# 10XGenomics/supernova

Hardware: AMD Instinct MI355X
Metric: Gk-mers/s through count+graph at k=48, 1.2B×150bp; bit-exact counts (higher is better)
Workload: dtype u64

## Files before the change

supernova_amd/csrc/snk_ctx.h:

```cpp
#pragma once
#include <hip/hip_runtime.h>
#include <stdarg.h>
#include <stdio.h>
#include <string.h>

#include <initializer_list>
#include <string>
#include <vector>

#include "../../include/snk.h"
#include "snk_launch.h"
#include "snk_opts.h"
#include "snk_plan.h"

struct snk_ctx {
    int device = 0;
    hipStream_t stream = nullptr;
    hipStream_t cur_stream = nullptr;
    int n_cu = 256;
    size_t lds_per_block = 65536;
    uint64_t device_mem_total = 0;
    double pass_sigma = 0.0;
    uint64_t plan_mapped = 0;
    uint64_t plan_mem = 0;
// ... 23 lines not shown
    uint32_t last_ovf = 0, last_ovf_nb = 0;
    uint64_t last_ovf_reads = 0;
    uint64_t last_dense = 0;
    uint32_t count_screen = 0;
    uint32_t count_tight = 0;
    snk_sizing_history sizing;
    uint32_t mlen = 16;
    uint32_t last_extra = 0;
    uint64_t last_input_fp = 0;
    bool have_input_fp = false;
    uint32_t last_count_limit = 0;
    uint32_t last_partition_passes = 1;
    uint32_t last_hbv_flood = 0;
    uint64_t last_hbv_dev_components = 0, last_hbv_host_components = 0;
    uint32_t last_bl_attempts = 0, last_bl_big_chunks = 0;
    uint64_t last_bl_circles = 0;
    std::vector<unsigned long long> h_region_off;
    snk_opts opts;
    void* shard = nullptr;
    void* host_io = nullptr;
    void (*host_io_free)(void*) = nullptr;
    void* df_io = nullptr;
    void (*df_io_free)(void*) = nullptr;
    void* stream_job = nullptr;
    void (*stream_job_free)(void*) = nullptr;
    void (*stream_job_invalidate)(void*) = nullptr;
    void* shard_host = nullptr;
    void (*shard_host_free)(void*) = nullptr;
};

// ... 54 lines not shown
```

supernova_amd/csrc/snk_dist.hip:

```cpp
#include <string.h>

#include <vector>

#include "snk_ctx.h"
#include "snk_common.h"
#include "snk_graph.h"
#include "snk_kernels.h"
#include "snk_stages.h"
#include "snk_shard.h"

static snk_shard_state* state_of(snk_ctx* ctx) { return snk_shard_state_of(ctx); }
void snk_shard_state_free(void* p) { delete static_cast<snk_shard_state*>(p); }
void snk_shard_state_invalidate_job(void* p) { if (p) static_cast<snk_shard_state*>(p)->job_open = false; }

int snk_shard_begin(snk_ctx* ctx, const snk_dev_reads* in, const snk_params* p, uint32_t rank, uint32_t world, uint32_t NB_total,
                    uint64_t* n_instances, hipStream_t st, char* err, size_t errcap) {
    if (!ctx || !in || !p) return snk_fail(SNK_E_ARG, err, errcap, "snk_shard_hist: NULL argument");
    if (p->K != 48 && p->K != 60) return snk_fail(SNK_E_UNSUPPORTED, err, errcap, "K=%u is not supported (48 or 60)", p->K);
    if (p->min_bc > 8) return snk_fail(SNK_E_UNSUPPORTED, err, errcap, "min_bc=%u: the device barcode rule tells up to eight distinct barcodes apart (min_bc <= 8)", p->min_bc);
    if (world == 0 || rank >= world || NB_total == 0 || NB_total % world) return snk_fail(SNK_E_ARG, err, errcap, "snk_shard_hist: NB_total must be a positive multiple of world");
    if (world > 0x7FFF) return snk_fail(SNK_E_UNSUPPORTED, err, errcap, "world > 32767");
    if (in->n_reads && (!in->rows || in->row_words * 16 < in->read_len || in->read_len > 256 || (!in->quals && !in->good_len)))
        return snk_fail(SNK_E_ARG, err, errcap, "snk_shard_hist: bad reads");
    SNK_HIP_TRY(snk_enter(ctx));
    snk_ctx_release_scratch(ctx);
    snk_shard_state* S = state_of(ctx);
    S->reads = *in;
    S->params = *p;
    S->rank = rank; S->world = world; S->NB_total = NB_total; S->NBl = NB_total / world;
    S->circ_all = nullptr; S->join_circles = 0;
    ctx->last_bl_attempts = ctx->last_bl_big_chunks = 0; ctx->last_bl_circles = 0;
    const uint16_t* good_len = (const uint16_t*)in->good_len;
    int rc;
    const bool fused = in->n_reads && snk_fused_trim_ok(ctx, in);
    snk_fused_trim ft;
    if (!good_len) {
        void* gl;
        if ((rc = snk_ctx_alloc(ctx, in->n_reads * 2 + 2, &gl, err, errcap))) return rc;
        if (fused) { ft.quals = in->quals; ft.qstride = in->qstride; ft.lens = in->lens; ft.min_qual = p->min_qual; ft.good_out = (uint16_t*)gl; }
        else if (in->n_reads) {
            rc = snk_dev_trim(ctx, in->quals, in->qstride, in->lens, in->read_len, in->n_reads, p->K, p->min_qual, gl, st);
            if (rc) return snk_fail(rc, err, errcap, "%s", snk_last_error());
        }
        good_len = (const uint16_t*)gl;
    }
    S->good_len = good_len;
// ... 13 lines not shown
int snk_shard_job_open(snk_ctx* ctx, const snk_params* p, uint32_t rank, uint32_t world, uint32_t NB_total, uint32_t read_len, uint64_t reads_ub,
                       uint64_t total_reads, int has_bc, hipStream_t st, char* err, size_t errcap) {
    if (!ctx || !p) return snk_fail(SNK_E_ARG, err, errcap, "snk_shard_stream_begin: NULL argument");
    if (p->K != 48 && p->K != 60) return snk_fail(SNK_E_UNSUPPORTED, err, errcap, "K=%u is not supported (48 or 60)", p->K);
    if (p->min_bc > 8) return snk_fail(SNK_E_UNSUPPORTED, err, errcap, "min_bc=%u: the device barcode rule tells up to eight distinct barcodes apart (min_bc <= 8)", p->min_bc);
    if (world == 0 || rank >= world || NB_total == 0 || NB_total % world) return snk_fail(SNK_E_ARG, err, errcap, "snk_shard_stream_begin: NB_total must be a positive multiple of world");
    if (read_len == 0 || read_len > 256 || reads_ub == 0) return snk_fail(SNK_E_ARG, err, errcap, "snk_shard_stream_begin: read_len 1..256 and an upper bound of this rank's reads are needed");
    SNK_HIP_TRY(snk_enter(ctx));
    snk_ctx_release_scratch(ctx);
    snk_shard_state* S = state_of(ctx);
    memset(&S->reads, 0, sizeof S->reads);
    S->params = *p;
    S->rank = rank; S->world = world; S->NB_total = NB_total; S->NBl = NB_total / world;
    S->circ_all = nullptr; S->join_circles = 0;
    ctx->last_bl_attempts = ctx->last_bl_big_chunks = 0; ctx->last_bl_circles = 0;
    S->job_open = false; S->job_read_len = read_len; S->job_has_bc = has_bc; S->job_reads_ub = reads_ub; S->job_total_reads = total_reads;
    void* q;
    int rc;
    if ((rc = snk_ctx_alloc(ctx, 64, &q, err, errcap))) return rc; S->status = (uint32_t*)q;
    SNK_HIP_TRY(hipMemsetAsync(S->status, 0, 64, st));
    if ((rc = snk_ctx_alloc(ctx, reads_ub * 2 + 64, &q, err, errcap))) return rc; S->job_good_len = (uint16_t*)q;
    const unsigned long long kpr = read_len >= p->K ? read_len - p->K + 1 : 0;
    if ((rc = snk_partition_open(ctx, st, p->K, NB_total, reads_ub * kpr, reads_ub, false, S->status, &S->job, err, errcap))) return rc;
    S->job_open = true;
    return SNK_OK;
}
int snk_shard_job_add(snk_ctx* ctx, const snk_dev_reads* slab, hipStream_t st, char* err, size_t errcap) {
    if (!ctx || !ctx->shard || !slab) return snk_fail(SNK_E_ARG, err, errcap, "snk_shard_stream_append: NULL argument / no open step");
    snk_shard_state* S = state_of(ctx);
    if (!S->job_open) return snk_fail(SNK_E_ARG, err, errcap, "snk_shard_stream_append: no open step (snk_shard_stream_begin)");
// ... 569 lines not shown
```

supernova_amd/csrc/snk_local.hip:

```cpp
#include <string.h>
#include <cstring>
#include <rocprim/rocprim.hpp>

#include <type_traits>

#include "snk_ctx.h"
#include "snk_common.h"
#include "snk_kernels.h"
#include "snk_graph.h"
#include "snk_stages.h"

namespace {

constexpr uint32_t NONE = 0xFFFFFFFFu;
constexpr unsigned long long NONE64 = ~0ull;
constexpr uint16_t NONE16 = 0xFFFFu;
constexpr int TB = 256;

struct chunk_src {
    const uint32_t* chunk_n;
    const uint32_t* chunk_base;
    const uint4* extra;
    const unsigned long long* region_off;
    uint32_t NB, n_extra, n_regions;
// ... 46 lines not shown
        const uint4 e = cs.extra[c - cs.NB];
        bucket = e.x; off = e.y; n = e.z & 0xFFFu; region = e.z >> 12; meta = e.w;
    }
    const uint64_t base = cs.region_off[region] + off;
    desc[c] = make_uint4((uint32_t)base, n, bucket, meta);
    if (desc_src) desc_src[c] = (uint64_t)region * region_cap + off;
}
__device__ __forceinline__ chunk_t chunk_get(const uint4* __restrict__ desc, uint32_t c) {
    const uint4 d = desc[c];
    chunk_t k;
    k.base = d.x; k.n = d.y; k.bucket = d.z; k.lg = d.w >> 24; k.id = d.w & 0xFFFFFFu; k.span = 1;
    if (d.w >> 31) { k.lg = 0; k.id = 0; k.span = d.w & 0xFFFFu; }
    return k;
}

__device__ __forceinline__ snk_kmer load_key(const snk_u128* keys, uint64_t i) {
    const uint64_t* p = reinterpret_cast<const uint64_t*>(keys + i);
    snk_kmer k;
    k.lo = p[0];
    k.hi = p[1];
    return k;
}
__device__ __forceinline__ uint32_t lhash(uint64_t hi, uint64_t lo) {
    uint32_t x = (uint32_t)(hi >> 32) * 0x9E3779B1u ^ (uint32_t)hi * 0x85EBCA77u ^ (uint32_t)(lo >> 32) * 0xC2B2AE3Du ^
                 (uint32_t)lo * 0x27D4EB2Fu;
    return snk_mix32(x);
}
template <int K>
__device__ __forceinline__ uint32_t oriented_base(snk_kmer k, bool rc, int idx) {
    return rc ? (snk_kmer_base<K>(k, K - 1 - idx) ^ 3u) : snk_kmer_base<K>(k, idx);
}

template <int K, int CAP, int T, bool BIG, bool GR, int MM>
__device__ __forceinline__ void bl_prune_chunk(const uint32_t c, const uint4* __restrict__ desc, uint32_t NB, bl_shard sh, const bl_regions& rg,
                                                     const snk_u128* __restrict__ keys, const uint64_t* __restrict__ vals,
                                                     uint32_t do_prune, uint8_t* __restrict__ ctx_out,
                                                     uint32_t* __restrict__ count_out, uint8_t* __restrict__ pend_out,
                                                     uint32_t* __restrict__ nbr_out, uint32_t* __restrict__ nbnd,
                                                     uint32_t* __restrict__ biglist, uint32_t* __restrict__ nbig,
                                                     unsigned long long* __restrict__ gindex, uint64_t gmask) {
    constexpr int HT = CAP <= 256 ? 512 : 4096;
    typedef typename std::conditional<(K <= 48 && !GR), uint32_t, uint64_t>::type klo_w;
    constexpr int KLS = (K <= 48 && !GR) ? 32 : 0;
    __shared__ uint64_t khi[CAP];
    __shared__ klo_w klo[CAP];
    __shared__ uint32_t ht[HT];
    __shared__ uint32_t bcnt;
    const int tid = threadIdx.x;
    const chunk_t ch = chunk_get(desc, c);
    if (ch.n == 0) return;
    if (!BIG && ch.n > (uint32_t)CAP) {
        if (tid == 0) biglist[atomicAdd(nbig, 1u)] = c;
        return;
    }
    const uint32_t n = ch.n;
// ... 23 lines not shown
            if (rg.keys_r) { uint64_t* d = reinterpret_cast<uint64_t*>(rg.keys_dense + ch.base + i); d[0] = kq[q].lo; d[1] = kq[q].hi; }
        }
    }
    __syncthreads();
    for (uint32_t i = tid; i < n; i += T) {
        uint32_t slot = lhash(khi[i], (uint64_t)klo[i] << KLS) & (HT - 1);
        for (;;) {
            const uint32_t old = atomicCAS(&ht[slot], 0u, i + 1u);
            if (old == 0u) break;
            slot = (slot + 1) & (HT - 1);
        }
    }
    __syncthreads();
    const uint32_t split_mask = (1u << ch.lg) - 1u;
    uint32_t mybnd = 0;
    __shared__ uint16_t mlist[8 * T];
    __shared__ uint32_t resL[T];
    __shared__ uint32_t mcnt;
#pragma unroll
    for (int q = 0; q < NPT; ++q) {
        const uint32_t i0 = q * T;
        if (i0 >= n) break;
        const uint32_t i = i0 + tid;
        const bool act = i < n;
        snk_kmer k;
        k.hi = act ? khi[i] : 0ull;
        k.lo = act ? ((uint64_t)klo[i] << KLS) : 0ull;
        uint64_t tag = 0;
        if (GR) { tag = k.lo & 0xFFFFFFFFull; k.lo &= ~0xFFFFFFFFull; }
        const uint64_t v = myv[q];
// ... 78 lines not shown
                    snk_kmer cn = snk_kmer_lt(r, y) ? r : y;
                    if (GR) cn.lo |= ktag;
                    uint32_t h1, h2;
                    snk_kmer_hash_count<(K > 48) || GR>(cn, &h1, &h2);
                    here = (h2 & split_mask) == ch.id;
                }
                if (here && !(do_prune & 2u)) { if (!(do_prune & 1u)) atomicOr(&resL[th], 1u << bit); }
                else atomicOr(&resL[th], (1u << bit) | (0x100u << bit) | (remote ? (0x10000u << bit) : 0u));
            }
        }
        __syncthreads();
        const uint32_t res = resL[tid];
        keep |= res & 0xFFu;
        const uint32_t pm = (res >> 8) & 0xFFu;
        __syncthreads();
        if (!act) continue;
        const uint64_t gi = ch.base + i;
        ctx_out[gi] = (uint8_t)keep;
        pend_out[gi] = (uint8_t)pm;
        if (sh.premote) sh.premote[gi] = (uint8_t)(res >> 16);
        count_out[gi] = (uint32_t)(v >> 8);
        nbr_out[gi] = (nb0 == NONE ? 0x0FFFu : nb0) | (snk_kmer_eq(k, kr) ? 0x8000u : 0u) | ((nb1 == NONE ? 0x0FFFu : nb1) << 16);
        if (pm) {
            ++mybnd;
            if (gindex) {
                snk_kmer kk;
                kk.hi = khi[i];
                kk.lo = (uint64_t)klo[i] << KLS;
                uint32_t h1, h2;
                snk_kmer_hash2(kk, &h1, &h2);
                uint64_t slot = (((uint64_t)h1 << 32) | h2) & gmask;
                const unsigned long long ent = ((unsigned long long)h1 << 32) | (unsigned long long)(gi + 1);
                if (gindex[gmask + 1] == 0ull) {
                    bool placed = false;
                    for (uint32_t tries = 0; tries < 64; ++tries) {
                        const unsigned long long old = atomicCAS(&gindex[slot], 0ull, ent);
                        if (old == 0ull) { placed = true; break; }
                        slot = (slot + 1) & gmask;
                    }
                    if (!placed) gindex[gmask + 1] = 1ull;
                }
            }
        }
    }
    snk_wave_add(&bcnt, mybnd);
    __syncthreads();
    if (tid == 0) nbnd[c] = bcnt;
}
template <int K, int CAP, int T, bool BIG, bool GR, int MM>
__global__ void __launch_bounds__(T) bl_prune_kernel(const uint4* __restrict__ desc, uint32_t NB, bl_shard sh, bl_regions rg, const uint32_t* __restrict__ biglist_in,
                                                     uint32_t nchunks, uint32_t cpw,
                                                     const snk_u128* __restrict__ keys, const uint64_t* __restrict__ vals,
                                                     uint32_t do_prune, uint8_t* __restrict__ ctx_out,
                                                     uint32_t* __restrict__ count_out, uint8_t* __restrict__ pend_out,
                                                     uint32_t* __restrict__ nbr_out, uint32_t* __restrict__ nbnd,
                                                     uint32_t* __restrict__ biglist, uint32_t* __restrict__ nbig, const uint32_t* __restrict__ n_dev,
                                                     unsigned long long* __restrict__ gindex, uint64_t gmask) {
    if (BIG && n_dev) {
        const uint32_t nb = *n_dev;
        for (uint32_t w = blockIdx.x; w < nb; w += gridDim.x)
            bl_prune_chunk<K, CAP, T, BIG, GR, MM>(biglist_in[w], desc, NB, sh, rg, keys, vals, do_prune, ctx_out, count_out, pend_out, nbr_out, nbnd, biglist, nbig, gindex, gmask);
        return;
    }
    for (uint32_t r = 0; r < cpw; ++r) {
        const uint32_t w = blockIdx.x * cpw + r;
        if (w >= nchunks) return;
        bl_prune_chunk<K, CAP, T, BIG, GR, MM>(BIG ? biglist_in[w] : w, desc, NB, sh, rg, keys, vals, do_prune, ctx_out, count_out, pend_out, nbr_out,
                                       nbnd, biglist, nbig, gindex, gmask);
    }
}

__global__ void __launch_bounds__(TB) bl_index_build_kernel(const snk_u128* __restrict__ keys, const uint8_t* __restrict__ pend,
                                                            uint64_t n, unsigned long long* __restrict__ tab, uint64_t mask) {
    const uint64_t i = (uint64_t)blockIdx.x * TB + threadIdx.x;
    if (i >= n || !pend[i]) return;
    const snk_kmer k = load_key(keys, i);
    uint32_t h1, h2;
    snk_kmer_hash2(k, &h1, &h2);
    uint64_t slot = (((uint64_t)h1 << 32) | h2) & mask;
    const unsigned long long ent = ((unsigned long long)h1 << 32) | (unsigned long long)(i + 1);
    for (;;) {
        const unsigned long long old = atomicCAS(&tab[slot], 0ull, ent);
        if (old == 0ull) break;
        slot = (slot + 1) & mask;
    }
}
template <int K, bool GR>
__global__ void __launch_bounds__(TB) bl_resolve_kernel(const snk_u128* __restrict__ keys, const uint8_t* __restrict__ pend,
                                                        uint64_t n, const unsigned long long* __restrict__ tab, uint64_t mask,
                                                        uint32_t do_prune, uint8_t* __restrict__ ctx, uint32_t* __restrict__ rq,
                                                        const uint8_t* __restrict__ premote) {
    constexpr int SPAN = 8 * TB;
    __shared__ uint16_t list[SPAN];
    __shared__ uint32_t cnt;
    const uint64_t base = (uint64_t)blockIdx.x * SPAN;
    if (threadIdx.x == 0) cnt = 0;
    __syncthreads();
    {
        const uint64_t i8 = base + 8ull * threadIdx.x;
        unsigned long long w = 0;
        if (i8 + 8 <= n) w = *reinterpret_cast<const unsigned long long*>(pend + i8);
        else for (uint64_t q = i8; q < n; ++q) w |= (unsigned long long)pend[q] << (8 * (q - i8));
        if (w) {
            uint32_t m = 0;
            for (int q = 0; q < 8; ++q) if ((w >> (8 * q)) & 0xFFull) ++m;
            uint32_t pos = atomicAdd(&cnt, m);
            for (int q = 0; q < 8; ++q) if ((w >> (8 * q)) & 0xFFull) list[pos++] = (uint16_t)(8 * threadIdx.x + q);
        }
    }
    __syncthreads();
    const uint32_t m = cnt;
    for (uint32_t it = threadIdx.x; it < m; it += TB) {
        const uint64_t i = base + list[it];
        const uint32_t pm = pend[i] & (premote ? ~(uint32_t)premote[i] : 0xFFu);
        snk_kmer k = load_key(keys, i);
        uint64_t tag = 0;
        if (GR) { tag = k.lo & 0xFFFFFFFFull; k.lo &= ~0xFFFFFFFFull; }
        uint32_t c = ctx[i];
        const snk_kmer kr = snk_kmer_rc<K>(k);
        for (uint32_t rem = pm; rem; rem &= rem - 1) {
            const uint32_t bit = __ffs(rem) - 1;
            const snk_kmer y = bit < 4 ? snk_kmer_succ<K>(k, bit) : snk_kmer_pred<K>(k, bit - 4);
            const snk_kmer r = bit < 4 ? snk_kmer_pred<K>(kr, 3u - bit) : snk_kmer_succ<K>(kr, 7u - bit);
            const bool rev = snk_kmer_lt(r, y);
            snk_kmer cy = rev ? r : y;
            if (GR) cy.lo |= tag;
            uint32_t h1, h2;
            snk_kmer_hash2(cy, &h1, &h2);
            uint64_t slot = (((uint64_t)h1 << 32) | h2) & mask;
            int64_t j = -1;
            for (;;) {
                const unsigned long long e = tab[slot];
                if (e == 0ull) break;
                if ((uint32_t)(e >> 32) == h1) {
                    const uint64_t idx = (uint32_t)e - 1u;
                    if (snk_kmer_eq(load_key(keys, idx), cy)) { j = (int64_t)idx; break; }
                }
                slot = (slot + 1) & mask;
            }
            if (j >= 0) rq[2 * i + (bit >> 2)] = ((uint32_t)j << 1) | (rev ? 1u : 0u);
            else if (do_prune) c &= ~(1u << bit);
            else rq[2 * i + (bit >> 2)] = NONE;
        }
        ctx[i] = (uint8_t)c;
    }
}

struct bl_extra_pool {
    unsigned long long* cur;
    uint64_t f0, b0;
    uint64_t fcap, bcap;
};
struct bl_dist_args {
    const uint8_t* premote;
    const uint32_t* rq_idx;
    const uint16_t* rq_meta;
    const unsigned long long* node_off;
    unsigned long long my_node_off;
};
template <int K, int CAP, int T, bool BIG, bool EMIT, bool DIST, bool GR>
// ... 420 lines not shown
    B->premote = nullptr;
    if (B->world > 1 || B->force_dist) {
        G_ALLOC(B->premote, uint8_t, n + 16);
        SNK_HIP_TRY(hipMemsetAsync(B->premote, 0, n + 16, st));
    }
    SNK_HIP_TRY(hipMemsetAsync(nbnd, 0, ((uint64_t)nchunks + 1) * 4, st));
    SNK_HIP_TRY(hipMemsetAsync(ctr, 0, 64, st));
    bl_shard sh;
    sh.bucket_base = B->premote ? B->rank * B->NBl : 0u;
    sh.NBl = B->premote ? B->NBl : 0u;
    sh.me = B->rank;
    sh.G = tab->n_regions ? tab->n_regions : 1u;
    sh.premote = B->premote;
    const uint32_t NBh = B->premote ? B->NB_total : tab->NB;
    const uint32_t cpw = snk_opt_u32(ctx, SNK_OPT_bl_cpw);
    uint64_t tg0 = 0;
    unsigned long long* index0 = nullptr;
    if (snk_opt_u32(ctx, SNK_OPT_bl_index_fused)) {
        const uint64_t guess = (ctx->last_bnd_n == n && ctx->last_bnd) ? ctx->last_bnd + ctx->last_bnd / 8 : n / 5;
        tg0 = 1024;
        while (tg0 < 2 * guess) tg0 <<= 1;
        G_ALLOC(index0, unsigned long long, tg0 + 1);
        SNK_HIP_TRY(hipMemsetAsync(index0, 0, (tg0 + 1) * 8, st));
    }
    bl_regions rg;
    rg.keys_r = tab->keys_r; rg.vals_r = tab->vals_r; rg.desc_src = desc_src;
    rg.keys_dense = const_cast<snk_u128*>(tab->keys);
    const bool long_m = ctx->mlen == (uint32_t)SNK_M_LONG;
    SNK_HIP_TRY(snk_launch(long_m ? bl_prune_kernel<K, SCAP, ST, false, GR, SNK_M_LONG> : bl_prune_kernel<K, SCAP, ST, false, GR, SNK_M_OF(K)>, snk_blocks(nchunks, cpw), ST, 0, st, (const uint4*)B->desc, NBh, sh, rg,
                           (const uint32_t*)nullptr, nchunks, cpw, tab->keys, tab->vals, B->do_prune | (snk_opt_u32(ctx, SNK_OPT_bl_noclassify) ? 2u : 0u), B->ctx, B->counts, B->pend, B->nbr, nbnd,
                           B->biglist, ctr, (const uint32_t*)nullptr, index0, tg0 - 1));
    uint32_t h_nbig = 0;
    SNK_HIP_TRY(hipMemcpyAsync(ctr + 1, ctr, 4, hipMemcpyDeviceToDevice, st));
    SNK_HIP_TRY(snk_launch(long_m ? bl_prune_kernel<K, BCAP, BT, true, GR, SNK_M_LONG> : bl_prune_kernel<K, BCAP, BT, true, GR, SNK_M_OF(K)>, 2048, BT, 0, st, (const uint4*)B->desc, NBh, sh, rg,
                           (const uint32_t*)B->biglist, 0u, 1u, tab->keys, tab->vals, B->do_prune | (snk_opt_u32(ctx, SNK_OPT_bl_noclassify) ? 2u : 0u), B->ctx, B->counts, B->pend, B->nbr,
                           nbnd, B->biglist, ctr + 2, (const uint32_t*)(ctr + 1), index0, tg0 - 1));
    if (tab->keys_r) {
        snk_ctx_release_block(ctx, tab->keys_r);
        snk_ctx_release_block(ctx, tab->vals_r);
    }
    unsigned long long* d_sum;
    G_ALLOC(d_sum, unsigned long long, 2);
    {
        size_t tb = 0;
        auto in = rocprim::make_transform_iterator(nbnd, [] __device__(uint32_t v) { return (unsigned long long)v; });
        SNK_HIP_TRY(rocprim::reduce((void*)nullptr, tb, in, d_sum, 0ull, (size_t)nchunks, rocprim::plus<unsigned long long>(), st));
        void* tmp;
        int rc = snk_ctx_alloc(ctx, tb, &tmp, err, errcap);
        if (rc) return rc;
        SNK_HIP_TRY(rocprim::reduce(tmp, tb, in, d_sum, 0ull, (size_t)nchunks, rocprim::plus<unsigned long long>(), st));
    }
    unsigned long long h_bnd = 0, h_gaveup = 0;
    if (index0) SNK_HIP_TRY(hipMemcpyAsync(&h_gaveup, index0 + tg0, 8, hipMemcpyDeviceToHost, st));
    SNK_HIP_TRY(hipMemcpyAsync(&h_bnd, d_sum, 8, hipMemcpyDeviceToHost, st));
    SNK_HIP_TRY(hipMemcpyAsync(&h_nbig, ctr + 1, 4, hipMemcpyDeviceToHost, st));
    SNK_HIP_TRY(snk_sync(st));
    B->nbig = h_nbig;
    B->n_boundary = h_bnd;
    ctx->last_bnd = h_bnd; ctx->last_bnd_n = n;
    uint64_t tg = 1024;
    while (tg < 2 * h_bnd) tg <<= 1;
    const bool fused_ok = index0 && !h_gaveup && h_bnd * 4 <= tg0 * 3;
    if (fused_ok) { B->index = index0; tg = tg0; }
    else {
        if (index0) snk_ctx_release_block(ctx, index0);
        G_ALLOC(B->index, unsigned long long, tg);
        SNK_HIP_TRY(hipMemsetAsync(B->index, 0, tg * 8, st));
    }
    B->index_mask = tg - 1;
    if (h_bnd) {
        if (!fused_ok) SNK_HIP_TRY(snk_launch(bl_index_build_kernel, snk_blocks(n, TB), TB, 0, st, tab->keys, B->pend, n, B->index, tg - 1));
        SNK_HIP_TRY(snk_launch(bl_resolve_kernel<K, GR>, snk_blocks(n, 8 * TB), TB, 0, st, tab->keys, B->pend, n,
                               B->index, tg - 1, B->do_prune, B->ctx, B->rq, (const uint8_t*)B->premote));
    }
    return SNK_OK;
}

template <int K, bool DIST, bool GR>
static int bl_fragments_impl(snk_ctx* ctx, hipStream_t st, snk_bl_state* B, const bl_dist_args& da, snk_frag_out* out, char* err,
                             size_t errcap) {
    const snk_table* tab = B->tab;
    const uint32_t nchunks = B->nchunks, h_nbig = B->nbig;
    uint32_t *nfrag, *foff;
    uint64_t *nbases, *boff;
    G_ALLOC(nfrag, uint32_t, (uint64_t)nchunks + 1);
    G_ALLOC(foff, uint32_t, (uint64_t)nchunks + 1);
    G_ALLOC(nbases, uint64_t, (uint64_t)nchunks + 1);
    G_ALLOC(boff, uint64_t, (uint64_t)nchunks + 1);
    SNK_HIP_TRY(hipMemsetAsync(nfrag, 0, ((uint64_t)nchunks + 1) * 4, st));
// ... 224 lines not shown
```

supernova_amd/csrc/snk_opts.hip:

```cpp
#include <stdio.h>
#include <stdlib.h>
#include <string.h>

#include <string>

#include "snk_opts.h"
#ifndef SNK_OPTS_NO_CTX
#include "snk_ctx.h"
#endif

const snk_opt_def snk_opt_defs[SNK_OPT_COUNT] = {
#define X(name, dflt, range, doc) {#name, dflt, range, doc},
    SNK_OPTIONS(X)
#undef X
};

int snk_opt_index(const char* name) {
    if (!name) return -1;
    for (int i = 0; i < SNK_OPT_COUNT; ++i) if (strcmp(snk_opt_defs[i].name, name) == 0) return i;
    return -1;
}
void snk_opts_init(snk_opts* o) { memset(o, 0, sizeof *o); }

int snk_opts_parse(snk_opts* o, const char* text, char* bad, unsigned badcap) {
// ... 135 lines not shown
    long long v;
    for (const tfield& f : tfields) if (get(f.opt, &v)) *reinterpret_cast<uint32_t*>(reinterpret_cast<char*>(t) + f.off) = (uint32_t)v;
    long long tight = 0, ng = 0;
    const bool ts = get(SNK_OPT_count_tight, &tight), ns = get(SNK_OPT_count_screen_ng, &ng);
    if (ns && ng >= 2) t->count_kernel = SNK_COUNT_KERNEL_SCREEN;
    else if (ts && tight) { t->count_kernel = SNK_COUNT_KERNEL_BOOKED; t->count_tight_slots = (uint32_t)tight; }
    else if (ts) t->count_kernel = SNK_COUNT_KERNEL_MARGIN;
    if (get(SNK_OPT_adaptive_buckets, &v)) t->adaptive_buckets = v ? 1 : 2;
    if (get(SNK_OPT_hot, &v)) t->hot_buckets = v ? 1 : 2;
    if (get(SNK_OPT_path_index, &v)) t->path_lookup = v ? 1 : 2;
    if (get(SNK_OPT_join_replicated, &v)) t->join_ranking = v ? 2 : 1;
    t->last_count_limit = ctx->last_count_limit;
    t->last_count_kernel = ctx->count_screen ? SNK_COUNT_KERNEL_SCREEN : (ctx->count_tight ? SNK_COUNT_KERNEL_BOOKED : SNK_COUNT_KERNEL_MARGIN);
    t->last_partition_passes = ctx->last_partition_passes;
    t->last_minimiser_len = ctx->mlen;
}
#endif
```

supernova_amd/csrc/snk_pipeline.hip:

```cpp
#include <string.h>
#include <cstring>
#include <rocprim/rocprim.hpp>

#include <stdlib.h>
#include <math.h>

#include <algorithm>
#include <vector>

#include "snk_ctx.h"
#include "snk_common.h"
#include "snk_graph.h"
#include "snk_kernels.h"
#include "snk_stages.h"

namespace {

__global__ void widen_offsets_kernel(const uint32_t* __restrict__ in, uint64_t* __restrict__ out, uint32_t n) {
    uint32_t i = blockIdx.x * blockDim.x + threadIdx.x;
    if (i < n) out[i] = in[i];
}

__global__ void __launch_bounds__(256) input_fp_kernel(const uint4* __restrict__ rows16, uint64_t n16, const uint4* __restrict__ aux16, uint64_t m16,
                                                       unsigned long long* __restrict__ out) {
// ... 27 lines not shown
        H.store(snk_sizing_key(K, grouped, ctx->mlen), n_reads, (ctx->count_screen && !grouped && H.screen_ratio > 0.0) ? H.screen_ratio : (double)tab.distinct / (double)h_ninst,
                (double)tab.n / (double)h_ninst);
    }
    snk_ctx_release_block(ctx, records);
    const uint64_t n_kmers = tab.n;
    out->buckets_split = tab.buckets_split;
    out->max_slots_used = tab.max_slots_used;
    out->n_kmers = n_kmers;
    out->keys = tab.keys;
    tm.mark();
    tm.mark();

    snk_graph_out go;
    ctx->last_bl_attempts = ctx->last_bl_big_chunks = 0;
    ctx->last_bl_circles = 0;
    if (local_graph) {
        snk_u128* keys_final = nullptr;
        rc = snk_local_graph(ctx, st, K, &tab, p->min_freq > 1 ? 1u : 0u, !(p->flags & SNK_F_NO_GRAPH),
                             !(p->flags & SNK_F_UNSORTED_TABLE), grouped, &go, &keys_final, out->graph_ms, err, errcap);
        if (rc) return rc;
        out->keys = keys_final;
        out->n_boundary = go.n_boundary;
        out->n_fragments = go.n_fragments;
    } else {
        rc = snk_graph_build(ctx, st, K, tab.keys, tab.vals, n_kmers, p->min_freq > 1 ? 1u : 0u, !(p->flags & SNK_F_NO_GRAPH), &go,
                             err, errcap);
        if (rc) return rc;
    }
    tm.mark();
    SNK_HIP_TRY(snk_sync(st));
// ... 400 lines not shown
```

supernova_amd/engine.py:

```python
from __future__ import annotations

import ctypes as C
from dataclasses import dataclass

import numpy as np
import torch

from . import lib as _lib
from .graphio import hbv_arrays

PHASES = ("trim", "plan", "partition", "count", "sort", "graph", "-", "total")


class DevArray:

    def __init__(self, ptr, *shape):
        self._ptr, self.shape = ptr, shape

    def data_ptr(self):
        return self._ptr


def _ptr(a):
    return a.data_ptr() if hasattr(a, "data_ptr") else a
# ... 291 lines not shown
            i += 1

    def set_tuning(self, **fields):
        t = _lib.SnkTuning()
        self.lib.snk_tuning_default(C.byref(t))
        for k, v in fields.items():
            if not hasattr(t, k) or k.startswith("last_") or k == "reserved":
                raise AttributeError(k)
            setattr(t, k, int(v))
        _lib.call(self.lib.snk_ctx_set_tuning, self._ctx, C.byref(t))

    def get_tuning(self) -> dict:
        t = _lib.SnkTuning()
        self.lib.snk_ctx_get_tuning(self._ctx, C.byref(t))
        return {k: int(getattr(t, k)) for k, _ in _lib.SnkTuning._fields_ if k != "reserved"}

    def reserve(self, n_bytes: int):
        _lib.call(self.lib.snk_ctx_reserve, self._ctx, int(n_bytes))

    def release_cache(self):
        self.lib.snk_ctx_trim(self._ctx)

    def close(self):
        if getattr(self, "_ctx", None):
            self.lib.snk_ctx_destroy(self._ctx)
            self._ctx = None

    def __del__(self):
        try:
            self.close()
# ... 290 lines not shown
```

Before: 97.75.

## Emit boundary records during prune and resolve from compact lists with wide index

The prune kernel now writes a compact record (key, position, pending and remote masks) for each boundary k-mer into hashed sublists. The index-build and resolve kernels then walk only these records instead of rescanning the whole pend array and reloading keys. A wide 16-byte index entry that stores the full key is added for K<=48, and slot selection uses a multiply-high instead of power-of-two masking, so probes can be checked without gathering the key from the table. If a sublist overflows, a scan-based record builder is used as a fallback; both paths cost extra memory for records and the wider index.

```diff
diff --git a/supernova_amd/csrc/snk_ctx.h b/supernova_amd/csrc/snk_ctx.h
--- a/supernova_amd/csrc/snk_ctx.h
+++ b/supernova_amd/csrc/snk_ctx.h
@@ -61,6 +61,7 @@
     uint32_t last_hbv_flood = 0;
     uint64_t last_hbv_dev_components = 0, last_hbv_host_components = 0;
     uint32_t last_bl_attempts = 0, last_bl_big_chunks = 0;
+    uint32_t last_bl_records = 0, last_bl_list_fallback = 0, last_bl_index_fallback = 0, last_bl_entry_bytes = 0;
     uint64_t last_bl_circles = 0;
     std::vector<unsigned long long> h_region_off;
     snk_opts opts;
diff --git a/supernova_amd/csrc/snk_dist.hip b/supernova_amd/csrc/snk_dist.hip
--- a/supernova_amd/csrc/snk_dist.hip
+++ b/supernova_amd/csrc/snk_dist.hip
@@ -30,6 +30,7 @@
     S->rank = rank; S->world = world; S->NB_total = NB_total; S->NBl = NB_total / world;
     S->circ_all = nullptr; S->join_circles = 0;
     ctx->last_bl_attempts = ctx->last_bl_big_chunks = 0; ctx->last_bl_circles = 0;
+    ctx->last_bl_records = ctx->last_bl_list_fallback = ctx->last_bl_index_fallback = ctx->last_bl_entry_bytes = 0;
     const uint16_t* good_len = (const uint16_t*)in->good_len;
     int rc;
     const bool fused = in->n_reads && snk_fused_trim_ok(ctx, in);
@@ -73,6 +74,7 @@
     S->rank = rank; S->world = world; S->NB_total = NB_total; S->NBl = NB_total / world;
     S->circ_all = nullptr; S->join_circles = 0;
     ctx->last_bl_attempts = ctx->last_bl_big_chunks = 0; ctx->last_bl_circles = 0;
+    ctx->last_bl_records = ctx->last_bl_list_fallback = ctx->last_bl_index_fallback = ctx->last_bl_entry_bytes = 0;
     S->job_open = false; S->job_read_len = read_len; S->job_has_bc = has_bc; S->job_reads_ub = reads_ub; S->job_total_reads = total_reads;
     void* q;
     int rc;
diff --git a/supernova_amd/csrc/snk_local.hip b/supernova_amd/csrc/snk_local.hip
--- a/supernova_amd/csrc/snk_local.hip
+++ b/supernova_amd/csrc/snk_local.hip
@@ -84,6 +84,48 @@
     return k;
 }
 
+constexpr uint32_t BL_REC_SUBLISTS = 1024, BL_REC_CUR_STRIDE = 32, BL_REC_SLACK = 64;
+static uint32_t bl_rec_sublists(uint64_t guess) {
+    uint32_t s = 1;
+    while (s < BL_REC_SUBLISTS && (uint64_t)s * 4096 <= guess) s <<= 1;
+    return s;
+}
+struct bl_bnd_out {
+    uint4* rec;
+    uint32_t* cur;
+    uint32_t cap_sub, nsub;
+    uint32_t sub_shift;
+    uint32_t wide;
+    uint64_t islots;
+};
+__device__ __forceinline__ uint32_t bl_rec_sublist(uint32_t unit, uint32_t shift) { return (uint32_t)((uint64_t)(unit * 0x9E3779B1u) >> shift); }
+__device__ __forceinline__ uint64_t bl_wide_slot(uint32_t h1, uint32_t h2, uint64_t islots) {
+    return __umul64hi(((uint64_t)h1 << 32) | h2, islots);
+}
+
+__device__ __forceinline__ bool bl_index_put(unsigned long long* __restrict__ tab, uint64_t mask, snk_kmer k, uint64_t pos, uint32_t limit) {
+    uint32_t h1, h2;
+    snk_kmer_hash2(k, &h1, &h2);
+    uint64_t slot = (((uint64_t)h1 << 32) | h2) & mask;
+    const unsigned long long ent = ((unsigned long long)h1 << 32) | (unsigned long long)(pos + 1);
+    for (uint32_t tries = 0; tries < limit; ++tries) {
+        if (atomicCAS(&tab[slot], 0ull, ent) == 0ull) return true;
+        slot = (slot + 1) & mask;
+    }
+    return false;
+}
+__device__ __forceinline__ bool bl_index_put_wide(unsigned long long* __restrict__ tab, uint64_t islots, snk_kmer k, uint64_t pos, uint32_t limit) {
+    uint32_t h1, h2;
+    snk_kmer_hash2(k, &h1, &h2);
+    uint64_t slot = bl_wide_slot(h1, h2, islots);
+    const unsigned long long w0 = (k.lo & ~0xFFFFFFFFull) | (unsigned long long)(pos + 1);
+    for (uint32_t tries = 0; tries < limit; ++tries) {
+        if (atomicCAS(&tab[2 * slot], 0ull, w0) == 0ull) { tab[2 * slot + 1] = k.hi; return true; }
+        if (++slot == islots) slot = 0;
+    }
+    return false;
+}
+
 __device__ __forceinline__ snk_kmer load_key(const snk_u128* keys, uint64_t i) {
     const uint64_t* p = reinterpret_cast<const uint64_t*>(keys + i);
     snk_kmer k;
@@ -108,7 +150,7 @@
                                                      uint32_t* __restrict__ count_out, uint8_t* __restrict__ pend_out,
                                                      uint32_t* __restrict__ nbr_out, uint32_t* __restrict__ nbnd,
                                                      uint32_t* __restrict__ biglist, uint32_t* __restrict__ nbig,
-                                                     unsigned long long* __restrict__ gindex, uint64_t gmask) {
+                                                     unsigned long long* __restrict__ gindex, uint64_t gmask, const bl_bnd_out& bo) {
     constexpr int HT = CAP <= 256 ? 512 : 4096;
     typedef typename std::conditional<(K <= 48 && !GR), uint32_t, uint64_t>::type klo_w;
     constexpr int KLS = (K <= 48 && !GR) ? 32 : 0;
@@ -162,6 +204,9 @@
     __syncthreads();
     const uint32_t split_mask = (1u << ch.lg) - 1u;
     uint32_t mybnd = 0;
+    uint32_t recm[NPT];
+#pragma unroll
+    for (int q = 0; q < NPT; ++q) recm[q] = 0;
     __shared__ uint16_t mlist[8 * T];
     __shared__ uint32_t resL[T];
     __shared__ uint32_t mcnt;
@@ -270,6 +315,7 @@
         keep |= res & 0xFFu;
         const uint32_t pm = (res >> 8) & 0xFFu;
         __syncthreads();
+        recm[q] = act ? (pm | (((res >> 16) & 0xFFu) << 8)) : 0u;
         if (!act) continue;
         const uint64_t gi = ch.base + i;
         ctx_out[gi] = (uint8_t)keep;
@@ -283,23 +329,38 @@
                 snk_kmer kk;
                 kk.hi = khi[i];
                 kk.lo = (uint64_t)klo[i] << KLS;
-                uint32_t h1, h2;
-                snk_kmer_hash2(kk, &h1, &h2);
-                uint64_t slot = (((uint64_t)h1 << 32) | h2) & gmask;
-                const unsigned long long ent = ((unsigned long long)h1 << 32) | (unsigned long long)(gi + 1);
-                if (gindex[gmask + 1] == 0ull) {
-                    bool placed = false;
-                    for (uint32_t tries = 0; tries < 64; ++tries) {
-                        const unsigned long long old = atomicCAS(&gindex[slot], 0ull, ent);
-                        if (old == 0ull) { placed = true; break; }
-                        slot = (slot + 1) & gmask;
-                    }
-                    if (!placed) gindex[gmask + 1] = 1ull;
+                const uint64_t flag = bo.wide ? 2 * bo.islots : gmask + 1;
+                if (gindex[flag] == 0ull) {
+                    const bool placed = bo.wide ? bl_index_put_wide(gindex, bo.islots, kk, gi, 64u) : bl_index_put(gindex, gmask, kk, gi, 64u);
+                    if (!placed) gindex[flag] = 1ull;
                 }
             }
         }
     }
-    snk_wave_add(&bcnt, mybnd);
+    const uint32_t incl = snk_wave_scan_incl(mybnd);
+    const uint32_t total = (uint32_t)__builtin_amdgcn_readlane((int)incl, 63);
+    if (total) {
+        const bool last = (tid & 63) == 63;
+        if (last) atomicAdd(&bcnt, total);
+        if (bo.rec) {
+            const uint32_t sub = bl_rec_sublist(c * (uint32_t)(T / 64) + ((uint32_t)tid >> 6), bo.sub_shift);
+            uint32_t at = 0;
+            if (last) at = atomicAdd(&bo.cur[sub * BL_REC_CUR_STRIDE], total);
+            at = (uint32_t)__builtin_amdgcn_readlane((int)at, 63) + incl - mybnd;
+            uint4* r = bo.rec + 2ull * (uint64_t)sub * bo.cap_sub;
+#pragma unroll
+            for (int q = 0; q < NPT; ++q) {
+                if ((recm[q] & 0xFFu) == 0u) continue;
+                if (at < bo.cap_sub) {
+                    const uint32_t i = tid + q * T;
+                    const uint64_t lo = (uint64_t)klo[i] << KLS, hi = khi[i];
+                    r[2ull * at] = make_uint4((uint32_t)lo, (uint32_t)(lo >> 32), (uint32_t)hi, (uint32_t)(hi >> 32));
+                    r[2ull * at + 1] = make_uint4((uint32_t)(ch.base + i), recm[q], 0u, 0u);
+                }
+                ++at;
+            }
+        }
+    }
     __syncthreads();
     if (tid == 0) nbnd[c] = bcnt;
 }
@@ -311,80 +372,127 @@
                                                      uint32_t* __restrict__ count_out, uint8_t* __restrict__ pend_out,
                                                      uint32_t* __restrict__ nbr_out, uint32_t* __restrict__ nbnd,
                                                      uint32_t* __restrict__ biglist, uint32_t* __restrict__ nbig, const uint32_t* __restrict__ n_dev,
-                                                     unsigned long long* __restrict__ gindex, uint64_t gmask) {
+                                                     unsigned long long* __restrict__ gindex, uint64_t gmask, bl_bnd_out bo) {
     if (BIG && n_dev) {
         const uint32_t nb = *n_dev;
         for (uint32_t w = blockIdx.x; w < nb; w += gridDim.x)
-            bl_prune_chunk<K, CAP, T, BIG, GR, MM>(biglist_in[w], desc, NB, sh, rg, keys, vals, do_prune, ctx_out, count_out, pend_out, nbr_out, nbnd, biglist, nbig, gindex, gmask);
+            bl_prune_chunk<K, CAP, T, BIG, GR, MM>(biglist_in[w], desc, NB, sh, rg, keys, vals, do_prune, ctx_out, count_out, pend_out, nbr_out, nbnd, biglist, nbig, gindex, gmask, bo);
         return;
     }
     for (uint32_t r = 0; r < cpw; ++r) {
         const uint32_t w = blockIdx.x * cpw + r;
         if (w >= nchunks) return;
         bl_prune_chunk<K, CAP, T, BIG, GR, MM>(BIG ? biglist_in[w] : w, desc, NB, sh, rg, keys, vals, do_prune, ctx_out, count_out, pend_out, nbr_out,
-                                       nbnd, biglist, nbig, gindex, gmask);
-    }
-}
-
-__global__ void __launch_bounds__(TB) bl_index_build_kernel(const snk_u128* __restrict__ keys, const uint8_t* __restrict__ pend,
-                                                            uint64_t n, unsigned long long* __restrict__ tab, uint64_t mask) {
-    const uint64_t i = (uint64_t)blockIdx.x * TB + threadIdx.x;
-    if (i >= n || !pend[i]) return;
-    const snk_kmer k = load_key(keys, i);
-    uint32_t h1, h2;
-    snk_kmer_hash2(k, &h1, &h2);
-    uint64_t slot = (((uint64_t)h1 << 32) | h2) & mask;
-    const unsigned long long ent = ((unsigned long long)h1 << 32) | (unsigned long long)(i + 1);
-    for (;;) {
-        const unsigned long long old = atomicCAS(&tab[slot], 0ull, ent);
-        if (old == 0ull) break;
-        slot = (slot + 1) & mask;
-    }
-}
-template <int K, bool GR>
-__global__ void __launch_bounds__(TB) bl_resolve_kernel(const snk_u128* __restrict__ keys, const uint8_t* __restrict__ pend,
-                                                        uint64_t n, const unsigned long long* __restrict__ tab, uint64_t mask,
-                                                        uint32_t do_prune, uint8_t* __restrict__ ctx, uint32_t* __restrict__ rq,
-                                                        const uint8_t* __restrict__ premote) {
-    constexpr int SPAN = 8 * TB;
-    __shared__ uint16_t list[SPAN];
+                                       nbnd, biglist, nbig, gindex, gmask, bo);
+    }
+}
+
+struct bl_rec_in {
+    const uint4* rec;
+    const uint32_t* cur;
+    uint32_t cur_stride, nsub, cap_sub, bps;
+};
+__device__ __forceinline__ const uint4* bl_rec_of_thread(const bl_rec_in& ri) {
+    const uint32_t sub = blockIdx.x / ri.bps, at = (blockIdx.x % ri.bps) * TB + threadIdx.x;
+    uint32_t m = ri.cur[(uint64_t)sub * ri.cur_stride];
+    if (m > ri.cap_sub) m = ri.cap_sub;
+    return at < m ? ri.rec + 2ull * ((uint64_t)sub * ri.cap_sub + at) : nullptr;
+}
+__device__ __forceinline__ snk_kmer bl_rec_key(uint4 a) {
+    snk_kmer k;
+    k.lo = ((uint64_t)a.y << 32) | a.x;
+    k.hi = ((uint64_t)a.w << 32) | a.z;
+    return k;
+}
+__global__ void __launch_bounds__(1024) bl_rec_close_kernel(const uint32_t* __restrict__ cur, uint32_t nsub, uint32_t cap_sub, uint32_t* __restrict__ out) {
+    __shared__ uint32_t total, over;
+    if (threadIdx.x == 0) { total = 0; over = 0; }
+    __syncthreads();
+    uint32_t m = 0, o = 0;
+    for (uint32_t s = threadIdx.x; s < nsub; s += 1024) {
+        const uint32_t c = cur[s * BL_REC_CUR_STRIDE];
+        m += c < cap_sub ? c : cap_sub;
+        o |= c > cap_sub ? 1u : 0u;
+    }
+    snk_wave_add(&total, m);
+    if (o) over = 1;
+    __syncthreads();
+    if (threadIdx.x == 0) { out[0] = total; out[1] = over; }
+}
+template <bool WRITE>
+__global__ void __launch_bounds__(TB) bl_records_build_kernel(const snk_u128* __restrict__ keys, const uint8_t* __restrict__ pend, const uint8_t* __restrict__ premote,
+                                                              uint64_t n, uint32_t* __restrict__ blk_cnt, const uint32_t* __restrict__ blk_off, uint4* __restrict__ rec) {
     __shared__ uint32_t cnt;
-    const uint64_t base = (uint64_t)blockIdx.x * SPAN;
     if (threadIdx.x == 0) cnt = 0;
     __syncthreads();
-    {
-        const uint64_t i8 = base + 8ull * threadIdx.x;
-        unsigned long long w = 0;
-        if (i8 + 8 <= n) w = *reinterpret_cast<const unsigned long long*>(pend + i8);
-        else for (uint64_t q = i8; q < n; ++q) w |= (unsigned long long)pend[q] << (8 * (q - i8));
-        if (w) {
-            uint32_t m = 0;
-            for (int q = 0; q < 8; ++q) if ((w >> (8 * q)) & 0xFFull) ++m;
-            uint32_t pos = atomicAdd(&cnt, m);
-            for (int q = 0; q < 8; ++q) if ((w >> (8 * q)) & 0xFFull) list[pos++] = (uint16_t)(8 * threadIdx.x + q);
-        }
-    }
-    __syncthreads();
-    const uint32_t m = cnt;
-    for (uint32_t it = threadIdx.x; it < m; it += TB) {
-        const uint64_t i = base + list[it];
-        const uint32_t pm = pend[i] & (premote ? ~(uint32_t)premote[i] : 0xFFu);
-        snk_kmer k = load_key(keys, i);
-        uint64_t tag = 0;
-        if (GR) { tag = k.lo & 0xFFFFFFFFull; k.lo &= ~0xFFFFFFFFull; }
-        uint32_t c = ctx[i];
-        const snk_kmer kr = snk_kmer_rc<K>(k);
-        for (uint32_t rem = pm; rem; rem &= rem - 1) {
-            const uint32_t bit = __ffs(rem) - 1;
-            const snk_kmer y = bit < 4 ? snk_kmer_succ<K>(k, bit) : snk_kmer_pred<K>(k, bit - 4);
-            const snk_kmer r = bit < 4 ? snk_kmer_pred<K>(kr, 3u - bit) : snk_kmer_succ<K>(kr, 7u - bit);
-            const bool rev = snk_kmer_lt(r, y);
-            snk_kmer cy = rev ? r : y;
-            if (GR) cy.lo |= tag;
-            uint32_t h1, h2;
-            snk_kmer_hash2(cy, &h1, &h2);
-            uint64_t slot = (((uint64_t)h1 << 32) | h2) & mask;
-            int64_t j = -1;
+    const uint64_t i8 = (uint64_t)blockIdx.x * (8 * TB) + 8ull * threadIdx.x;
+    unsigned long long w = 0;
+    if (i8 + 8 <= n) w = *reinterpret_cast<const unsigned long long*>(pend + i8);
+    else for (uint64_t q = i8; q < n; ++q) w |= (unsigned long long)pend[q] << (8 * (q - i8));
+    uint32_t m = 0;
+    for (int q = 0; q < 8; ++q) if ((w >> (8 * q)) & 0xFFull) ++m;
+    uint32_t pos = snk_wave_alloc(&cnt, m);
+    if (WRITE) {
+        pos += blk_off[blockIdx.x];
+        for (int q = 0; q < 8; ++q) {
+            const uint32_t pm = (uint32_t)(w >> (8 * q)) & 0xFFu;
+            if (!pm) continue;
+            const uint64_t i = i8 + q;
+            const snk_kmer k = load_key(keys, i);
+            rec[2ull * pos] = make_uint4((uint32_t)k.lo, (uint32_t)(k.lo >> 32), (uint32_t)k.hi, (uint32_t)(k.hi >> 32));
+            rec[2ull * pos + 1] = make_uint4((uint32_t)i, pm | ((premote ? (uint32_t)premote[i] : 0u) << 8), 0u, 0u);
+            ++pos;
+        }
+        return;
+    }
+    __syncthreads();
+    if (threadIdx.x == 0) blk_cnt[blockIdx.x] = cnt;
+}
+template <bool WIDE>
+__global__ void __launch_bounds__(TB) bl_index_build_kernel(bl_rec_in ri, unsigned long long* __restrict__ tab, uint64_t size) {
+    const uint4* r = bl_rec_of_thread(ri);
+    if (!r) return;
+    const snk_kmer k = bl_rec_key(r[0]);
+    const uint64_t pos = r[1].x;
+    if (WIDE) bl_index_put_wide(tab, size, k, pos, 0xFFFFFFFFu);
+    else bl_index_put(tab, size - 1, k, pos, 0xFFFFFFFFu);
+}
+template <int K, bool GR, bool WIDE>
+__global__ void __launch_bounds__(TB) bl_resolve_kernel(bl_rec_in ri, const snk_u128* __restrict__ keys, const unsigned long long* __restrict__ tab,
+                                                        uint64_t size , uint32_t do_prune, uint8_t* __restrict__ ctx,
+                                                        uint32_t* __restrict__ rq) {
+    static_assert(!WIDE || (K <= 48 && !GR), "whole-key entries need the low 32 key bits");
+    const uint4* rp = bl_rec_of_thread(ri);
+    if (!rp) return;
+    const uint4 ra = rp[0], rb = rp[1];
+    snk_kmer k = bl_rec_key(ra);
+    const uint64_t i = rb.x;
+    const uint32_t pm = rb.y & 0xFFu & ~(rb.y >> 8);
+    uint64_t tag = 0;
+    if (GR) { tag = k.lo & 0xFFFFFFFFull; k.lo &= ~0xFFFFFFFFull; }
+    uint32_t gone = 0;
+    const snk_kmer kr = snk_kmer_rc<K>(k);
+    for (uint32_t rem = pm; rem; rem &= rem - 1) {
+        const uint32_t bit = __ffs(rem) - 1;
+        const snk_kmer y = bit < 4 ? snk_kmer_succ<K>(k, bit) : snk_kmer_pred<K>(k, bit - 4);
+        const snk_kmer r = bit < 4 ? snk_kmer_pred<K>(kr, 3u - bit) : snk_kmer_succ<K>(kr, 7u - bit);
+        const bool rev = snk_kmer_lt(r, y);
+        snk_kmer cy = rev ? r : y;
+        if (GR) cy.lo |= tag;
+        uint32_t h1, h2;
+        snk_kmer_hash2(cy, &h1, &h2);
+        int64_t j = -1;
+        if (WIDE) {
+            const uint4* wt = reinterpret_cast<const uint4*>(tab);
+            uint64_t slot = bl_wide_slot(h1, h2, size);
+            for (;;) {
+                const uint4 e = wt[slot];
+                if (e.x == 0u) break;
+                if (e.y == (uint32_t)(cy.lo >> 32) && e.z == (uint32_t)cy.hi && e.w == (uint32_t)(cy.hi >> 32)) { j = (int64_t)(e.x - 1u); break; }
+                if (++slot == size) slot = 0;
+            }
+        } else {
+            uint64_t slot = (((uint64_t)h1 << 32) | h2) & size;
             for (;;) {
                 const unsigned long long e = tab[slot];
                 if (e == 0ull) break;
@@ -392,14 +500,14 @@
                     const uint64_t idx = (uint32_t)e - 1u;
                     if (snk_kmer_eq(load_key(keys, idx), cy)) { j = (int64_t)idx; break; }
                 }
-                slot = (slot + 1) & mask;
+                slot = (slot + 1) & size;
             }
-            if (j >= 0) rq[2 * i + (bit >> 2)] = ((uint32_t)j << 1) | (rev ? 1u : 0u);
-            else if (do_prune) c &= ~(1u << bit);
-            else rq[2 * i + (bit >> 2)] = NONE;
-        }
-        ctx[i] = (uint8_t)c;
-    }
+        }
+        if (j >= 0) rq[2 * i + (bit >> 2)] = ((uint32_t)j << 1) | (rev ? 1u : 0u);
+        else if (do_prune) gone |= 1u << bit;
+        else rq[2 * i + (bit >> 2)] = NONE;
+    }
+    if (gone) ctx[i] = (uint8_t)(ctx[i] & ~gone);
 }
 
 struct bl_extra_pool {
@@ -850,27 +958,41 @@
     sh.premote = B->premote;
     const uint32_t NBh = B->premote ? B->NB_total : tab->NB;
     const uint32_t cpw = snk_opt_u32(ctx, SNK_OPT_bl_cpw);
+    constexpr bool CAN_WIDE = K <= 48 && !GR;
+    const bool wide = CAN_WIDE && !B->premote;
+    const uint64_t guess = (ctx->last_bnd_n == n && ctx->last_bnd) ? ctx->last_bnd + ctx->last_bnd / 8 : n / 5;
     uint64_t tg0 = 0;
     unsigned long long* index0 = nullptr;
     if (snk_opt_u32(ctx, SNK_OPT_bl_index_fused)) {
-        const uint64_t guess = (ctx->last_bnd_n == n && ctx->last_bnd) ? ctx->last_bnd + ctx->last_bnd / 8 : n / 5;
         tg0 = 1024;
-        while (tg0 < 2 * guess) tg0 <<= 1;
-        G_ALLOC(index0, unsigned long long, tg0 + 1);
-        SNK_HIP_TRY(hipMemsetAsync(index0, 0, (tg0 + 1) * 8, st));
-    }
+        if (wide) tg0 = std::max<uint64_t>(tg0, 2 * guess);
+        else while (tg0 < 2 * guess) tg0 <<= 1;
+        const uint64_t words = wide ? 2 * tg0 + 2 : tg0 + 1;
+        G_ALLOC(index0, unsigned long long, words);
+        SNK_HIP_TRY(hipMemsetAsync(index0, 0, words * 8, st));
+    }
+    bl_bnd_out bo;
+    bo.nsub = bl_rec_sublists(guess);
+    bo.sub_shift = 32u - (uint32_t)__builtin_ctz(bo.nsub);
+    bo.cap_sub = (uint32_t)(guess / bo.nsub) + BL_REC_SLACK;
+    bo.wide = wide ? 1u : 0u;
+    bo.islots = tg0;
+    G_ALLOC(bo.rec, uint4, 2ull * bo.nsub * bo.cap_sub);
+    G_ALLOC(bo.cur, uint32_t, BL_REC_SUBLISTS * BL_REC_CUR_STRIDE);
+    SNK_HIP_TRY(hipMemsetAsync(bo.cur, 0, BL_REC_SUBLISTS * BL_REC_CUR_STRIDE * 4, st));
     bl_regions rg;
     rg.keys_r = tab->keys_r; rg.vals_r = tab->vals_r; rg.desc_src = desc_src;
     rg.keys_dense = const_cast<snk_u128*>(tab->keys);
     const bool long_m = ctx->mlen == (uint32_t)SNK_M_LONG;
     SNK_HIP_TRY(snk_launch(long_m ? bl_prune_kernel<K, SCAP, ST, false, GR, SNK_M_LONG> : bl_prune_kernel<K, SCAP, ST, false, GR, SNK_M_OF(K)>, snk_blocks(nchunks, cpw), ST, 0, st, (const uint4*)B->desc, NBh, sh, rg,
                            (const uint32_t*)nullptr, nchunks, cpw, tab->keys, tab->vals, B->do_prune | (snk_opt_u32(ctx, SNK_OPT_bl_noclassify) ? 2u : 0u), B->ctx, B->counts, B->pend, B->nbr, nbnd,
-                           B->biglist, ctr, (const uint32_t*)nullptr, index0, tg0 - 1));
+                           B->biglist, ctr, (const uint32_t*)nullptr, index0, tg0 - 1, bo));
     uint32_t h_nbig = 0;
     SNK_HIP_TRY(hipMemcpyAsync(ctr + 1, ctr, 4, hipMemcpyDeviceToDevice, st));
     SNK_HIP_TRY(snk_launch(long_m ? bl_prune_kernel<K, BCAP, BT, true, GR, SNK_M_LONG> : bl_prune_kernel<K, BCAP, BT, true, GR, SNK_M_OF(K)>, 2048, BT, 0, st, (const uint4*)B->desc, NBh, sh, rg,
                            (const uint32_t*)B->biglist, 0u, 1u, tab->keys, tab->vals, B->do_prune | (snk_opt_u32(ctx, SNK_OPT_bl_noclassify) ? 2u : 0u), B->ctx, B->counts, B->pend, B->nbr,
-                           nbnd, B->biglist, ctr + 2, (const uint32_t*)(ctr + 1), index0, tg0 - 1));
+                           nbnd, B->biglist, ctr + 2, (const uint32_t*)(ctr + 1), index0, tg0 - 1, bo));
+    SNK_HIP_TRY(snk_launch(bl_rec_close_kernel, 1, 1024, 0, st, (const uint32_t*)bo.cur, bo.nsub, bo.cap_sub, ctr + 4));
     if (tab->keys_r) {
         snk_ctx_release_block(ctx, tab->keys_r);
         snk_ctx_release_block(ctx, tab->vals_r);
@@ -887,28 +1009,63 @@
         SNK_HIP_TRY(rocprim::reduce(tmp, tb, in, d_sum, 0ull, (size_t)nchunks, rocprim::plus<unsigned long long>(), st));
     }
     unsigned long long h_bnd = 0, h_gaveup = 0;
-    if (index0) SNK_HIP_TRY(hipMemcpyAsync(&h_gaveup, index0 + tg0, 8, hipMemcpyDeviceToHost, st));
+    uint32_t h_ctr[5] = {0, 0, 0, 0, 0};
+    if (index0) SNK_HIP_TRY(hipMemcpyAsync(&h_gaveup, index0 + (wide ? 2 * tg0 : tg0), 8, hipMemcpyDeviceToHost, st));
     SNK_HIP_TRY(hipMemcpyAsync(&h_bnd, d_sum, 8, hipMemcpyDeviceToHost, st));
-    SNK_HIP_TRY(hipMemcpyAsync(&h_nbig, ctr + 1, 4, hipMemcpyDeviceToHost, st));
+    SNK_HIP_TRY(hipMemcpyAsync(h_ctr, ctr + 1, sizeof h_ctr, hipMemcpyDeviceToHost, st));
     SNK_HIP_TRY(snk_sync(st));
+    h_nbig = h_ctr[0];
+    const uint32_t h_rec[2] = {h_ctr[3], h_ctr[4]};
     B->nbig = h_nbig;
     B->n_boundary = h_bnd;
     ctx->last_bnd = h_bnd; ctx->last_bnd_n = n;
     uint64_t tg = 1024;
-    while (tg < 2 * h_bnd) tg <<= 1;
+    if (wide) tg = std::max<uint64_t>(tg, 2 * h_bnd);
+    else while (tg < 2 * h_bnd) tg <<= 1;
     const bool fused_ok = index0 && !h_gaveup && h_bnd * 4 <= tg0 * 3;
     if (fused_ok) { B->index = index0; tg = tg0; }
     else {
         if (index0) snk_ctx_release_block(ctx, index0);
-        G_ALLOC(B->index, unsigned long long, tg);
-        SNK_HIP_TRY(hipMemsetAsync(B->index, 0, tg * 8, st));
+        G_ALLOC(B->index, unsigned long long, wide ? 2 * tg : tg);
+        SNK_HIP_TRY(hipMemsetAsync(B->index, 0, (wide ? 2 * tg : tg) * 8, st));
     }
     B->index_mask = tg - 1;
+    bl_rec_in ri;
+    ri.rec = bo.rec; ri.cur = bo.cur; ri.cur_stride = BL_REC_CUR_STRIDE; ri.nsub = bo.nsub; ri.cap_sub = bo.cap_sub;
+    const bool list_ok = !h_rec[1];
+    if (!list_ok && h_bnd) {
+        const uint64_t nblk = snk_blocks(n, 8 * TB);
+        uint32_t *blk_cnt, *blk_off;
+        G_ALLOC(blk_cnt, uint32_t, nblk + 1);
+        G_ALLOC(blk_off, uint32_t, nblk + 1);
+        snk_ctx_release_block(ctx, bo.rec);
+        uint4* rec2;
+        G_ALLOC(rec2, uint4, 2ull * h_bnd);
+        SNK_HIP_TRY(snk_launch(bl_records_build_kernel<false>, nblk, TB, 0, st, tab->keys, (const uint8_t*)B->pend, (const uint8_t*)B->premote, n, blk_cnt,
+                               (const uint32_t*)nullptr, (uint4*)nullptr));
+        int rc = excl_scan<uint32_t>(ctx, st, blk_cnt, blk_off, (size_t)nblk, err, errcap);
+        if (rc) return rc;
+        SNK_HIP_TRY(snk_launch(bl_records_build_kernel<true>, nblk, TB, 0, st, tab->keys, (const uint8_t*)B->pend, (const uint8_t*)B->premote, n, (uint32_t*)nullptr,
+                               (const uint32_t*)blk_off, rec2));
+        ri.rec = rec2; ri.cur = reinterpret_cast<const uint32_t*>(d_sum); ri.cur_stride = 0; ri.nsub = 1; ri.cap_sub = (uint32_t)h_bnd;
+    }
+    ri.bps = (uint32_t)snk_blocks(ri.cap_sub, TB);
+    ctx->last_bl_records = list_ok ? h_rec[0] : (uint32_t)h_bnd;
+    ctx->last_bl_list_fallback = list_ok ? 0u : 1u;
+    ctx->last_bl_index_fallback = fused_ok ? 0u : 1u;
+    ctx->last_bl_entry_bytes = wide ? 16u : 8u;
     if (h_bnd) {
-        if (!fused_ok) SNK_HIP_TRY(snk_launch(bl_index_build_kernel, snk_blocks(n, TB), TB, 0, st, tab->keys, B->pend, n, B->index, tg - 1));
-        SNK_HIP_TRY(snk_launch(bl_resolve_kernel<K, GR>, snk_blocks(n, 8 * TB), TB, 0, st, tab->keys, B->pend, n,
-                               B->index, tg - 1, B->do_prune, B->ctx, B->rq, (const uint8_t*)B->premote));
-    }
+        const uint64_t grid = (uint64_t)ri.nsub * ri.bps;
+        if (!fused_ok) {
+            if (wide) SNK_HIP_TRY(snk_launch(bl_index_build_kernel<true>, grid, TB, 0, st, ri, B->index, tg));
+            else SNK_HIP_TRY(snk_launch(bl_index_build_kernel<false>, grid, TB, 0, st, ri, B->index, tg));
+        }
+        if constexpr (CAN_WIDE) {
+            if (wide) SNK_HIP_TRY(snk_launch(bl_resolve_kernel<K, GR, true>, grid, TB, 0, st, ri, tab->keys, (const unsigned long long*)B->index, tg, B->do_prune, B->ctx, B->rq));
+        }
+        if (!wide) SNK_HIP_TRY(snk_launch(bl_resolve_kernel<K, GR, false>, grid, TB, 0, st, ri, tab->keys, (const unsigned long long*)B->index, tg - 1, B->do_prune, B->ctx, B->rq));
+    }
+    snk_ctx_release_block(ctx, const_cast<uint4*>(ri.rec));
     return SNK_OK;
 }
 
diff --git a/supernova_amd/csrc/snk_opts.hip b/supernova_amd/csrc/snk_opts.hip
--- a/supernova_amd/csrc/snk_opts.hip
+++ b/supernova_amd/csrc/snk_opts.hip
@@ -173,5 +173,9 @@
     t->last_count_kernel = ctx->count_screen ? SNK_COUNT_KERNEL_SCREEN : (ctx->count_tight ? SNK_COUNT_KERNEL_BOOKED : SNK_COUNT_KERNEL_MARGIN);
     t->last_partition_passes = ctx->last_partition_passes;
     t->last_minimiser_len = ctx->mlen;
+    t->reserved[5] = ctx->last_bl_records;
+    t->reserved[6] = ctx->last_bl_list_fallback;
+    t->reserved[7] = ctx->last_bl_index_fallback;
+    t->reserved[8] = ctx->last_bl_entry_bytes;
 }
 #endif
diff --git a/supernova_amd/csrc/snk_pipeline.hip b/supernova_amd/csrc/snk_pipeline.hip
--- a/supernova_amd/csrc/snk_pipeline.hip
+++ b/supernova_amd/csrc/snk_pipeline.hip
@@ -65,6 +65,7 @@
     snk_graph_out go;
     ctx->last_bl_attempts = ctx->last_bl_big_chunks = 0;
     ctx->last_bl_circles = 0;
+    ctx->last_bl_records = ctx->last_bl_list_fallback = ctx->last_bl_index_fallback = ctx->last_bl_entry_bytes = 0;
     if (local_graph) {
         snk_u128* keys_final = nullptr;
         rc = snk_local_graph(ctx, st, K, &tab, p->min_freq > 1 ? 1u : 0u, !(p->flags & SNK_F_NO_GRAPH),
diff --git a/supernova_amd/engine.py b/supernova_amd/engine.py
--- a/supernova_amd/engine.py
+++ b/supernova_amd/engine.py
@@ -329,6 +329,11 @@
         t = _lib.SnkTuning()
         self.lib.snk_ctx_get_tuning(self._ctx, C.byref(t))
         return {k: int(getattr(t, k)) for k, _ in _lib.SnkTuning._fields_ if k != "reserved"}
+
+    def last_boundary_resolve(self) -> dict:
+        t = _lib.SnkTuning()
+        self.lib.snk_ctx_get_tuning(self._ctx, C.byref(t))
+        return {"records": int(t.reserved[5]), "list_fallback": int(t.reserved[6]), "index_fallback": int(t.reserved[7]), "entry_bytes": int(t.reserved[8])}
 
     def reserve(self, n_bytes: int):
         _lib.call(self.lib.snk_ctx_reserve, self._ctx, int(n_bytes))
```

Result: no change. 98.09, median of 3 (+0.3%).
